# kkaitlyn111/cs336-a2-systems

Measured on AMD Instinct MI355X. Metric: tokens/sec/node GPT-2-XL bf16 DDP, higher is better.
Workload: dtype bf16; 1 GPU; global_batch=102, per_gpu_batch=102, seq_len=512, parallelism=dp1, ddp=none, optimizer=fused HIP AdamW (fp32 master weights), overlapped with backward, attention=HIP FlashAttention-2 (causal), hip_graph=False, gemm_selection=per-problem fastest of hipblaslt default / autotuned lt_gemm / cs336 MFMA GEMM

## Files before the change

csrc/bindings.cpp:

```cpp
#include <ATen/ATen.h>
#include <ATen/hip/HIPContext.h>
#include <c10/core/DeviceGuard.h>
#include <torch/library.h>

#include <algorithm>
#include <cstdlib>
#include <cstring>
#include <mutex>
#include <string>
#include <unordered_map>
#include <vector>

#include "cs336/kernels.h"
#include "../gemm/gemm8.h"

namespace {

using cs336::DType;

DType to_dtype(const at::Tensor& t) {
  switch (t.scalar_type()) {
    case at::kFloat: return DType::F32;
    case at::kBFloat16: return DType::BF16;
    case at::kHalf: return DType::F16;
// ... 903 lines not shown
    TORCH_CHECK(aligned(p) && aligned(g) && aligned(m) && aligned(v) && aligned(s) && aligned(w),
                "cs336: adamw_step_t pointers must be 16-byte aligned");
    const at::Tensor* ts[6] = {&p, &g, &m, &v, &s, &w};
    for (int k = 0; k < 6; ++k) h[(int64_t)i * 6 + k] = reinterpret_cast<int64_t>(ts[k]->data_ptr());
    h[(int64_t)n * 6 + i] = tiles;
    tiles += ((R + 255) / 256) * ((C + 63) / 64);
    int64_t* d = h + (int64_t)n * 6 + (n + 1) + 3 * i;
    d[0] = R;
    d[1] = C;
    d[2] = w.stride(0);
  }
  h[(int64_t)n * 6 + n] = tiles;
  c10::DeviceGuard guard(params[0].device());
  at::Tensor dev = device_table(hv, params[0].device());
  const int64_t* dptr = dev.data_ptr<int64_t>();
  const double alpha_t = lr * (std::sqrt(1.0 - std::pow(beta2, (double)step)) / (1.0 - std::pow(beta1, (double)step)));
  cs336::adamw_step_t(dptr, dptr + (int64_t)n * 6, dptr + (int64_t)n * 6 + (n + 1), n, tiles, to_dtype(grads[0]),
                      (float)beta1, (float)beta2, (float)(1.0 - beta1), (float)(1.0 - beta2), (float)eps,
                      (float)(lr * weight_decay), (float)alpha_t, alpha_ptr(alpha_dev, params[0]), stream());
}

void multi_tensor_cast_bf16(std::vector<at::Tensor> src, std::vector<at::Tensor> dst) {
  if (src.empty()) return;
  check_same_dtype(src, at::kFloat, "src");
  check_same_dtype(dst, at::kBFloat16, "dst");
  c10::DeviceGuard g(src[0].device());
  HostTable ht = build_table({src, dst});
  cs336::multi_tensor_cast_bf16(ht.tt, stream());
}

at::Tensor multi_tensor_l2norm(std::vector<at::Tensor> tensors) {
  TORCH_CHECK(!tensors.empty(), "cs336: empty tensor list");
  const at::ScalarType st = tensors[0].scalar_type();
  check_same_dtype(tensors, st, "tensors");
  c10::DeviceGuard g(tensors[0].device());
  HostTable ht = build_table({tensors});
  at::Tensor partials = at::empty({std::max<int64_t>(ht.tt.total_chunks, 1)}, tensors[0].options().dtype(at::kFloat));
  at::Tensor out = at::zeros({}, tensors[0].options().dtype(at::kFloat));
  cs336::multi_tensor_sumsq(ht.tt, to_dtype(tensors[0]), partials.data_ptr<float>(), stream());
  cs336::finalize_l2norm(partials.data_ptr<float>(), ht.tt.total_chunks, out.data_ptr<float>(), stream());
  return out;
}

void multi_tensor_scale_(std::vector<at::Tensor> tensors, const at::Tensor& scale) {
  if (tensors.empty()) return;
  const at::ScalarType st = tensors[0].scalar_type();
  check_same_dtype(tensors, st, "tensors");
  TORCH_CHECK(scale.scalar_type() == at::kFloat && scale.numel() == 1 && scale.is_cuda(), "cs336: scale");
  c10::DeviceGuard g(tensors[0].device());
  HostTable ht = build_table({tensors});
  cs336::multi_tensor_scale(ht.tt, to_dtype(tensors[0]), scale.data_ptr<float>(), stream());
}

}

void occupy(int64_t n_workgroups, int64_t lds_bytes, double ms, at::Tensor& counter) {
  check_cuda(counter, "counter");
  TORCH_CHECK(counter.scalar_type() == at::kInt && counter.numel() >= 1, "cs336: occupy counter must be int32");
  TORCH_CHECK(n_workgroups > 0 && n_workgroups <= 65536 && lds_bytes >= 4 && lds_bytes <= 160 * 1024 && ms >= 0 &&
                  ms <= 10000,
              "cs336: occupy arguments out of range");
  cs336::occupy((int)n_workgroups, (int)lds_bytes, ms, counter.data_ptr<int>(), stream());
}

void occupy_bytes(int64_t n_workgroups, int64_t lds_bytes, double ms, const at::Tensor& src, at::Tensor& dst,
                  int64_t total_bytes, at::Tensor& counter) {
  check_cuda(src, "src");
  TORCH_CHECK(counter.scalar_type() == at::kInt && counter.numel() >= 1, "cs336: occupy counter must be int32");
  const int64_t nb = src.numel() * src.element_size();
  TORCH_CHECK(src.is_contiguous() && dst.is_contiguous() && dst.numel() * dst.element_size() >= nb && nb >= 16384,
              "cs336: occupy_bytes needs contiguous src/dst of >= 16 KiB, dst at least src's size");
  TORCH_CHECK(n_workgroups > 0 && n_workgroups <= 4096 && lds_bytes >= 4 && lds_bytes <= 65536 && ms > 0 && ms < 10000 &&
                  total_bytes >= 0,
              "cs336: occupy_bytes arguments out of range");
  c10::DeviceGuard g(src.device());
  cs336::occupy_bytes((int)n_workgroups, (int)lds_bytes, ms, src.data_ptr(), dst.data_ptr(), nb & ~(int64_t)16383,
                      total_bytes, counter.data_ptr<int>(), stream());
}

void cohort(int64_t n_workgroups, int64_t lds_bytes, double deadline_ms, at::Tensor& state) {
  check_cuda(state, "state");
  TORCH_CHECK(state.scalar_type() == at::kInt && state.numel() >= 3 && state.is_contiguous(),
              "cs336: cohort state must be a contiguous int32[3]");
  TORCH_CHECK(n_workgroups > 0 && n_workgroups <= 4096 && lds_bytes >= 4 && lds_bytes <= 160 * 1024 &&
                  deadline_ms > 0 && deadline_ms <= 2000,
              "cs336: cohort arguments out of range");
  cs336::cohort((int)n_workgroups, (int)lds_bytes, deadline_ms, state.data_ptr<int>(), stream());
}

bool gemm8_check(const at::Tensor& t, int64_t rows, int64_t cols, const char* what) {
  TORCH_CHECK(t.is_cuda() && t.scalar_type() == at::kBFloat16 && t.dim() == 2 && t.stride(1) == 1, "cs336: gemm8 ",
              what, " must be a row-major bf16 CUDA matrix");
  TORCH_CHECK(t.size(0) == rows && t.size(1) == cols, "cs336: gemm8 ", what, " shape ", t.sizes(), " expected (", rows,
              ", ", cols, ")");
  TORCH_CHECK(t.stride(0) % 8 == 0 && reinterpret_cast<uintptr_t>(t.data_ptr()) % 16 == 0, "cs336: gemm8 ", what,
              " rows must be 16-B aligned");
  return true;
}

bool gemm8_ok(int64_t M, int64_t N, int64_t K, int64_t epi, int64_t half) {
  if (M <= 0 || N <= 0 || K <= 0 || M >= (1 << 30) || N >= (1 << 30) || K >= (1 << 30)) return false;
  const int fn = cs336::gemm8::pick_fn((int)N, (int)epi, (int)half);
  if (fn == 0 || M % 256) return false;
  if (epi == 0) return N % 8 == 0 && K % 8 == 0;
  return K % 64 == 0 && N % (64 * fn) == 0 && (epi != 3 || half % (64 * fn) == 0);
}

constexpr int64_t kDmaLimit = (int64_t(1) << 31) - (int64_t(1) << 20);
bool gemm8_extents_ok(const at::Tensor& a, const at::Tensor& b) {
  const int64_t K = a.size(1);
  return (255 * a.stride(0) + K) * 2 < kDmaLimit && ((b.size(0) - 1) * b.stride(0) + K) * 2 < kDmaLimit;
}

void gemm8(const at::Tensor& a, const at::Tensor& b, at::Tensor& c, int64_t epi, int64_t fn, const OptT& h,
           const OptT& y, int64_t half) {
  const int64_t M = a.size(0), K = a.size(1), N = b.size(0);
  gemm8_check(a, M, K, "a");
  gemm8_check(b, N, K, "b");
  TORCH_CHECK(epi >= 0 && epi <= 2, "cs336: gemm8 epi");
  TORCH_CHECK(gemm8_ok(M, N, K, epi, half), "cs336: gemm8 does not take M=", M, " N=", N, " K=", K, " epi=", epi);
  TORCH_CHECK(gemm8_extents_ok(a, b), "cs336: gemm8 operand extent exceeds the 2 GiB DMA range");
  cs336::gemm8::Args p{};
  p.a = reinterpret_cast<const uint16_t*>(a.data_ptr());
  p.b = reinterpret_cast<const uint16_t*>(b.data_ptr());
  p.lda = a.stride(0);
  p.ldb = b.stride(0);
  p.M = (int)M;
  p.N = (int)N;
  p.K = (int)K;
  p.half = (int)half;
  if (epi == 0) {
    gemm8_check(c, M, N, "c");
  } else if (epi == 1) {
    TORCH_CHECK(N == 2 * half, "cs336: gemm8 epi 1 needs b = [w1; w3] with 2·half rows");
    gemm8_check(c, M, N, "y");
    TORCH_CHECK(h.has_value() && h->defined(), "cs336: gemm8 epi 1 needs h");
    gemm8_check(*h, M, half, "h");
    p.h = reinterpret_cast<uint16_t*>(h->data_ptr());
    p.ldh = h->stride(0);
  } else {
    TORCH_CHECK(N == half, "cs336: gemm8 epi 2 needs b with half rows");
    gemm8_check(c, M, 2 * half, "c = [da|db]");
    TORCH_CHECK(y.has_value() && y->defined(), "cs336: gemm8 epi 2 needs y");
    gemm8_check(*y, M, 2 * half, "y");
    p.y = reinterpret_cast<const uint16_t*>(y->data_ptr());
    p.ldy = y->stride(0);
  }
  p.c = reinterpret_cast<uint16_t*>(c.data_ptr());
  p.ldc = c.stride(0);
  c10::DeviceGuard g(a.device());
  TORCH_CHECK(cs336::gemm8::launch(p, (int)epi, (int)fn, stream()), "cs336: gemm8 launch (fn ", fn, ")");
}

bool gemm8_stamps(const std::optional<at::Tensor>& buf) {
  if (!buf.has_value()) return cs336::gemm8::set_stamp_buffer(nullptr, 0);
  const at::Tensor& b = *buf;
  TORCH_CHECK(b.is_cuda() && b.scalar_type() == at::kLong && b.is_contiguous() && b.dim() == 2 && b.size(1) == 8,
              "cs336: gemm8 stamp buffer must be a contiguous int64 (blocks, 8) GPU tensor");
  return cs336::gemm8::set_stamp_buffer(reinterpret_cast<uint64_t*>(b.data_ptr<int64_t>()), b.size(0));
}

void gemm8_rope(const at::Tensor& a, const at::Tensor& b, at::Tensor& c, const at::Tensor& cos, const at::Tensor& sin,
                const OptT& pos, int64_t seq, int64_t rope_cols, int64_t dhead) {
  const int64_t M = a.size(0), K = a.size(1), N = b.size(0);
  gemm8_check(a, M, K, "a");
  gemm8_check(b, N, K, "b");
  gemm8_check(c, M, N, "c");
  TORCH_CHECK(gemm8_ok(M, N, K, 3, rope_cols), "cs336: gemm8_rope does not take M=", M, " N=", N, " K=", K,
              " rope_cols=", rope_cols);
  TORCH_CHECK(gemm8_extents_ok(a, b), "cs336: gemm8_rope operand extent exceeds the 2 GiB DMA range");
  TORCH_CHECK(dhead % 8 == 0 && dhead > 0 && dhead <= 96 && rope_cols % dhead == 0 && rope_cols <= N && seq > 0,
              "cs336: gemm8_rope needs d_head % 8 == 0, d_head <= 96 and whole rotated heads");
  TORCH_CHECK(cos.is_cuda() && sin.is_cuda() && cos.scalar_type() == at::kFloat && sin.scalar_type() == at::kFloat &&
                  cos.is_contiguous() && sin.is_contiguous() && cos.dim() == 2 && cos.size(1) == dhead / 2 &&
                  sin.sizes() == cos.sizes(),
              "cs336: gemm8_rope cos/sin must be contiguous fp32 (ctx, d_head/2)");
  const int64_t* pp = nullptr;
  if (pos.has_value() && pos->defined()) {
    TORCH_CHECK(pos->is_cuda() && pos->scalar_type() == at::kLong && pos->is_contiguous() && pos->numel() == M,
                "cs336: gemm8_rope pos must be contiguous int64 with one entry per row");
    pp = pos->data_ptr<int64_t>();
  } else {
    TORCH_CHECK(seq <= cos.size(0), "cs336: gemm8_rope seq ", seq, " exceeds the RoPE cache ", cos.size(0));
  }
  cs336::gemm8::Args p{};
  p.a = reinterpret_cast<const uint16_t*>(a.data_ptr());
  p.b = reinterpret_cast<const uint16_t*>(b.data_ptr());
  p.c = reinterpret_cast<uint16_t*>(c.data_ptr());
  p.lda = a.stride(0);
  p.ldb = b.stride(0);
  p.ldc = c.stride(0);
  p.M = (int)M;
  p.N = (int)N;
  p.K = (int)K;
  p.rcos = cos.data_ptr<float>();
  p.rsin = sin.data_ptr<float>();
  p.rpos = pp;
  p.rseq = (int)seq;
  p.rope_cols = (int)rope_cols;
  p.rdh = (int)dhead;
  c10::DeviceGuard g(a.device());
  TORCH_CHECK(cs336::gemm8::launch(p, 3, 0, stream()), "cs336: gemm8_rope launch");
}

void gemm8w(const at::Tensor& a, const at::Tensor& b, at::Tensor& out, int64_t splits, bool trans_out,
            bool accumulate, int64_t fn) {
  TORCH_CHECK(a.is_cuda() && b.is_cuda() && a.scalar_type() == at::kBFloat16 && b.scalar_type() == at::kBFloat16 &&
                  a.dim() == 2 && b.dim() == 2 && a.stride(1) == 1 && b.stride(1) == 1,
              "cs336: gemm8w needs row-major bf16 CUDA operands");
  const int64_t K = a.size(0), M = a.size(1), N = b.size(1);
  TORCH_CHECK(b.size(0) == K, "cs336: gemm8w contraction mismatch");
  TORCH_CHECK(a.stride(0) % 8 == 0 && b.stride(0) % 8 == 0 && reinterpret_cast<uintptr_t>(a.data_ptr()) % 16 == 0 &&
                  reinterpret_cast<uintptr_t>(b.data_ptr()) % 16 == 0 && M % 8 == 0 && N % 8 == 0,
              "cs336: gemm8w needs 16-B aligned rows");
  TORCH_CHECK(out.is_cuda() && out.scalar_type() == at::kFloat, "cs336: gemm8w out must be fp32 CUDA");
  const int64_t rows = trans_out ? N : M, cols = trans_out ? M : N;
  if (splits > 1) {
    TORCH_CHECK(out.dim() == 3 && out.size(0) == splits && out.size(1) == rows && out.size(2) == cols &&
                    out.is_contiguous() && !accumulate,
                "cs336: gemm8w split-K out must be contiguous (splits, rows, cols) slabs");
  } else {
    TORCH_CHECK(out.dim() == 2 && out.size(0) == rows && out.size(1) == cols && out.stride(1) == 1 &&
                    out.stride(0) % 4 == 0 && reinterpret_cast<uintptr_t>(out.data_ptr()) % 16 == 0,
                "cs336: gemm8w out shape/alignment");
  }
  TORCH_CHECK(K % 64 == 0 && K > 0, "cs336: gemm8w needs K % 64 == 0");
  const int64_t ld = std::max(a.stride(0), b.stride(0)), wide = std::max(M, N);
  auto extent = [&](int64_t rows) { return rows * ld * 2 + wide * 2; };
  const int64_t nkt = K / 64, per_split = (nkt + splits - 1) / splits * 64;
  TORCH_CHECK(splits == 1 || extent(per_split) < kDmaLimit, "cs336: gemm8w split of ", per_split,
              " token rows exceeds the 2 GiB DMA range; use more splits (", splits, " given)");
  const int64_t chunk = std::max<int64_t>(64, std::min(K, (kDmaLimit - wide * 2) / (ld * 2) / 64 * 64));
  TORCH_CHECK(splits > 1 || extent(chunk) < kDmaLimit, "cs336: gemm8w rows too wide for the DMA range");
  c10::DeviceGuard g(a.device());
  for (int64_t k0 = 0; k0 < K; k0 += (splits > 1 ? K : chunk)) {
    const int64_t kc = splits > 1 ? K : std::min(chunk, K - k0);
    cs336::gemm8::WArgs p{};
    p.a = reinterpret_cast<const uint16_t*>(a.data_ptr()) + k0 * a.stride(0);
    p.b = reinterpret_cast<const uint16_t*>(b.data_ptr()) + k0 * b.stride(0);
    p.c = out.data_ptr<float>();
    p.lda = a.stride(0);
    p.ldb = b.stride(0);
    p.ldc = splits > 1 ? cols : out.stride(0);
    p.slab_stride = splits > 1 ? rows * cols : 0;
    p.a_elems = (kc - 1) * a.stride(0) + M;
    p.b_elems = (kc - 1) * b.stride(0) + N;
    p.M = (int)M;
    p.N = (int)N;
    p.K = (int)kc;
    p.splits = (int)splits;
    p.trans_out = trans_out ? 1 : 0;
    p.accumulate = (accumulate || k0 > 0) ? 1 : 0;
    TORCH_CHECK(cs336::gemm8::launch_w(p, (int)fn, stream()), "cs336: gemm8w does not take M=", M, " N=", N,
                " K=", kc, " splits=", splits);
  }
}

void splitk_sum(const at::Tensor& slabs, at::Tensor& out, bool accumulate) {
  TORCH_CHECK(slabs.is_cuda() && slabs.scalar_type() == at::kFloat && slabs.dim() == 3 && slabs.is_contiguous(),
              "cs336: splitk_sum slabs must be contiguous fp32 (splits, M, N)");
  const int64_t M = slabs.size(1), N = slabs.size(2);
  TORCH_CHECK(out.is_cuda() && out.scalar_type() == at::kFloat && out.dim() == 2 && out.size(0) == M &&
                  out.size(1) == N && out.stride(1) == 1 && out.stride(0) % 4 == 0 && N % 4 == 0 &&
                  reinterpret_cast<uintptr_t>(out.data_ptr()) % 16 == 0,
              "cs336: splitk_sum out must be fp32 (M, N) with 16-B aligned rows");
  if (M * N == 0 || slabs.size(0) == 0) return;
  c10::DeviceGuard g(slabs.device());
  cs336::gemm::splitk_reduce(slabs.data_ptr<float>(), out.data_ptr<float>(), M, N, (int)slabs.size(0), out.stride(0),
                             accumulate, stream());
}

void check_cache(const at::Tensor& t, const char* name) {
  check_cuda(t, name);
  TORCH_CHECK(t.dim() == 4, "cs336: ", name, " must be (B, H, max_len, D)");
  TORCH_CHECK(t.stride(3) == 1, "cs336: ", name, " must have a contiguous last dim");
  const int64_t es = t.element_size();
  TORCH_CHECK((reinterpret_cast<uintptr_t>(t.data_ptr()) % 16) == 0, "cs336: ", name, " must be 16-byte aligned");
  TORCH_CHECK((t.stride(2) * es) % 16 == 0 && (t.stride(1) * es) % 16 == 0 && (t.stride(0) * es) % 16 == 0,
              "cs336: ", name, " strides must be multiples of 16 bytes");
  TORCH_CHECK(t.stride(0) >= 0 && t.stride(1) >= 0 && t.stride(2) >= t.size(3), "cs336: ", name,
              " rows must not overlap");
  TORCH_CHECK(t.size(2) < ((int64_t)1 << 31), "cs336: ", name, " max_len must fit 32 bits");
}

std::tuple<at::Tensor, at::Tensor> fa_decode(const at::Tensor& q, const at::Tensor& k_cache, const at::Tensor& v_cache,
                                             const at::Tensor& kv_len, double scale, int64_t max_kv_len,
                                             int64_t splits) {
  check_cuda(q, "q");
  check_cache(k_cache, "k_cache");
  check_cache(v_cache, "v_cache");
  TORCH_CHECK(q.dim() == 3, "cs336: fa_decode q must be (B, H, D)");
  const int64_t B = q.size(0), H = q.size(1), D = q.size(2), max_len = k_cache.size(2);
  TORCH_CHECK(D == 32 || D == 64 || D == 80 || D == 128, "cs336: fa_decode head dim must be 32, 64, 80 or 128 (got ", D,
              ")");
  TORCH_CHECK(q.scalar_type() == k_cache.scalar_type() && q.scalar_type() == v_cache.scalar_type(),
              "cs336: q / k_cache / v_cache dtype mismatch");
  TORCH_CHECK(k_cache.sizes() == v_cache.sizes() && k_cache.size(0) == B && k_cache.size(1) == H &&
                  k_cache.size(3) == D,
              "cs336: caches must be (B, H, max_len, D) matching q");
  TORCH_CHECK(k_cache.device() == q.device() && v_cache.device() == q.device() && kv_len.device() == q.device(),
              "cs336: fa_decode tensors must be on one device");
  TORCH_CHECK(kv_len.scalar_type() == at::kInt && kv_len.dim() == 1 && kv_len.size(0) == B && kv_len.is_contiguous(),
              "cs336: kv_len must be a contiguous int32 (B,) device tensor");
  TORCH_CHECK(max_kv_len >= 0 && max_kv_len <= max_len, "cs336: max_kv_len must be in [0, max_len]");
  TORCH_CHECK(splits >= 0 && splits <= 64, "cs336: splits must be in [0, 64] (0 = choose)");
  TORCH_CHECK(B * H * 64 < ((int64_t)1 << 31), "cs336: fa_decode grid too large");
  const DType t = to_dtype(q);
  c10::DeviceGuard g(q.device());
  const at::Tensor qc = q.contiguous();
  TORCH_CHECK((reinterpret_cast<uintptr_t>(qc.data_ptr()) % 16) == 0, "cs336: q must be 16-byte aligned");
  at::Tensor o = at::empty({B, H, D}, q.options());
  at::Tensor lse = at::empty({B, H}, q.options().dtype(at::kFloat));
  if (B * H == 0) return {o, lse};
  cs336::DecodeParams p;
  p.q = qc.data_ptr();
  p.k = k_cache.data_ptr();
  p.v = v_cache.data_ptr();
  p.o = o.data_ptr();
  p.lse = lse.data_ptr<float>();
  p.kv_len = kv_len.data_ptr<int>();
  p.k_sb = k_cache.stride(0); p.k_sh = k_cache.stride(1); p.k_sn = k_cache.stride(2);
  p.v_sb = v_cache.stride(0); p.v_sh = v_cache.stride(1); p.v_sn = v_cache.stride(2);
  p.B = (int)B; p.H = (int)H; p.D = (int)D; p.max_len = (int)max_len;
  p.scale = (float)scale;
  p.splits = splits > 0 ? (int)splits : cs336::fa_decode_splits((int)B, (int)H, (int)D, t, (int)max_kv_len);
  at::Tensor ws;
  if (p.splits > 1) {
    ws = at::empty({(int64_t)p.splits * B * H * (D + 1)}, q.options().dtype(at::kFloat));
    p.opart = ws.data_ptr<float>();
    p.lpart = p.opart + (int64_t)p.splits * B * H * D;
  }
  cs336::fa_decode(p, t, stream());
  return {o, lse};
}

int64_t fa_decode_splits(int64_t B, int64_t H, int64_t D, int64_t elem_size, int64_t max_kv_len) {
  return cs336::fa_decode_splits((int)B, (int)H, (int)D, elem_size == 4 ? DType::F32 : DType::BF16, (int)max_kv_len);
}

at::Tensor kv_append_rope(const at::Tensor& qkv, const at::Tensor& cos, const at::Tensor& sin, const at::Tensor& pos,
                          at::Tensor& k_cache, at::Tensor& v_cache) {
  check_cuda(qkv, "qkv");
  check_cache(k_cache, "k_cache");
  check_cache(v_cache, "v_cache");
  TORCH_CHECK(qkv.dim() == 2 && qkv.stride(1) == 1, "cs336: qkv must be (B, 3*H*D) with a contiguous last dim");
  const int64_t B = k_cache.size(0), H = k_cache.size(1), max_len = k_cache.size(2), D = k_cache.size(3);
  TORCH_CHECK(k_cache.sizes() == v_cache.sizes(), "cs336: k_cache / v_cache shape mismatch");
  TORCH_CHECK(qkv.size(0) == B && qkv.size(1) == 3 * H * D, "cs336: qkv must be (B, 3*H*D) for (B, H, max_len, D) caches");
  TORCH_CHECK(D >= 8 && D <= 256 && D % 8 == 0, "cs336: kv_append_rope head dim must be a multiple of 8 in [8, 256]");
  TORCH_CHECK(qkv.scalar_type() == k_cache.scalar_type() && qkv.scalar_type() == v_cache.scalar_type(),
              "cs336: qkv / k_cache / v_cache dtype mismatch");
  TORCH_CHECK((reinterpret_cast<uintptr_t>(qkv.data_ptr()) % 16) == 0 && (qkv.stride(0) * qkv.element_size()) % 16 == 0 &&
                  qkv.stride(0) >= 0,
              "cs336: qkv rows must be 16-byte aligned");
  TORCH_CHECK(cos.is_cuda() && sin.is_cuda() && cos.scalar_type() == at::kFloat && sin.scalar_type() == at::kFloat &&
                  cos.dim() == 2 && cos.is_contiguous() && sin.is_contiguous() && cos.sizes() == sin.sizes() &&
                  cos.size(1) * 2 == D,
              "cs336: rope cache must be contiguous fp32 (ctx, D/2)");
  TORCH_CHECK(pos.scalar_type() == at::kInt && pos.dim() == 1 && pos.size(0) == B && pos.is_contiguous(),
              "cs336: pos must be a contiguous int32 (B,) device tensor");
  TORCH_CHECK(pos.device() == qkv.device() && cos.device() == qkv.device() && sin.device() == qkv.device() &&
                  k_cache.device() == qkv.device() && v_cache.device() == qkv.device(),
              "cs336: kv_append_rope tensors must be on one device");
  TORCH_CHECK(B * 3 * H * (D / 8) < ((int64_t)1 << 31) && cos.size(0) < ((int64_t)1 << 31),
              "cs336: kv_append_rope too large for 32-bit indexing");
  c10::DeviceGuard g(qkv.device());
  at::Tensor q_out = at::empty({B, H, D}, qkv.options());
  if (B * H == 0) return q_out;
  cs336::AppendParams p;
  p.qkv = qkv.data_ptr();
  p.qkv_sb = qkv.stride(0);
  p.cos = cos.data_ptr<float>();
  p.sin = sin.data_ptr<float>();
  p.pos = pos.data_ptr<int>();
  p.q_out = q_out.data_ptr();
  p.k = k_cache.data_ptr();
  p.v = v_cache.data_ptr();
  p.k_sb = k_cache.stride(0); p.k_sh = k_cache.stride(1); p.k_sn = k_cache.stride(2);
  p.v_sb = v_cache.stride(0); p.v_sh = v_cache.stride(1); p.v_sn = v_cache.stride(2);
  p.B = (int)B; p.H = (int)H; p.D = (int)D; p.max_len = (int)max_len; p.ctx = (int)cos.size(0);
  cs336::kv_append_rope(p, to_dtype(qkv), stream());
  return q_out;
}

bool gemm_skinny_ok(int64_t M, int64_t N, int64_t K, int64_t elem_size) {
  return cs336::gemm_skinny_ok(M, N, K, elem_size);
}

void gemm_skinny(const at::Tensor& x, const at::Tensor& w, at::Tensor& out) {
  check_cuda(x, "x");
  check_cuda(w, "w");
  check_cuda(out, "out");
  TORCH_CHECK(x.dim() == 2 && w.dim() == 2 && out.dim() == 2, "cs336: gemm_skinny takes x (M, K), w (N, K), out (M, N)");
  TORCH_CHECK(x.scalar_type() == at::kBFloat16 || x.scalar_type() == at::kHalf, "cs336: gemm_skinny takes bf16 / fp16");
  TORCH_CHECK(w.scalar_type() == x.scalar_type() && out.scalar_type() == x.scalar_type(),
              "cs336: gemm_skinny x / w / out dtype mismatch");
  TORCH_CHECK(w.device() == x.device() && out.device() == x.device(), "cs336: gemm_skinny tensors must be on one device");
  const int64_t M = x.size(0), K = x.size(1), N = w.size(0);
  TORCH_CHECK(w.size(1) == K && out.size(0) == M && out.size(1) == N, "cs336: gemm_skinny shape mismatch");
  TORCH_CHECK(M >= 1 && M <= 16, "cs336: gemm_skinny takes 1 <= M <= 16 (got ", M, ")");
  TORCH_CHECK(K >= 8 && K % 8 == 0, "cs336: gemm_skinny needs K % 8 == 0 (got ", K, ")");
  TORCH_CHECK(cs336::gemm_skinny_ok(M, N, K, x.element_size()), "cs336: gemm_skinny extents exceed the kernel's 32-bit row / k indices");
  TORCH_CHECK(x.stride(1) == 1 && w.stride(1) == 1 && out.stride(1) == 1, "cs336: gemm_skinny operands must have a contiguous last dim");
  TORCH_CHECK(x.stride(0) % 8 == 0 && (M == 1 || x.stride(0) >= 0), "cs336: gemm_skinny x row stride must be a non-negative multiple of 8");
  TORCH_CHECK(w.stride(0) % 8 == 0 && (N == 1 || w.stride(0) >= K), "cs336: gemm_skinny w row stride must be a multiple of 8, at least K");
// ... 133 lines not shown
```

csrc/gemm/gemm8.h:

```cpp
#pragma once

#include <hip/hip_runtime.h>
#include <stdint.h>

namespace cs336 {
namespace gemm8 {

struct Args {
  const uint16_t* a;
  const uint16_t* b;
  uint16_t* c;
  uint16_t* h;
  const uint16_t* y;
  int64_t lda, ldb, ldc, ldh, ldy;
  int M, N, K;
  int half;
  const float* rcos;
  const float* rsin;
  const int64_t* rpos;
  int rseq, rope_cols, rdh;
  uint64_t* stamps = nullptr;
};
int pick_fn(int N, int epi, int half);
bool set_stamp_buffer(uint64_t* buf, int64_t blocks);
bool launch(const Args& p, int epi, int fn, hipStream_t s);

struct WArgs {
  const uint16_t* a;
  const uint16_t* b;
  float* c;
  int64_t lda, ldb, ldc, slab_stride;
  int64_t a_elems, b_elems;
  int M, N, K;
  int splits;
  int trans_out, accumulate;
};
bool launch_w(const WArgs& p, int fn, hipStream_t s);

}
}
```

csrc/gemm/gemm8w.hip:

```cpp
#include "cs336/kernels.h"
#include "gemm8.h"

namespace cs336 {
namespace gemm8 {
namespace {

typedef __attribute__((ext_vector_type(8))) __bf16 bf16x8;
typedef __attribute__((ext_vector_type(4))) float f32x4;
typedef __attribute__((ext_vector_type(4))) short s16x4;
typedef __attribute__((ext_vector_type(8))) short s16x8;
typedef __attribute__((address_space(3))) s16x4 lds_s16x4;
typedef __attribute__((address_space(3))) void* lds_ptr_t;

constexpr int BM = 256, BK = 64, NT = 512;
constexpr int kGroupM = 8;

__device__ __forceinline__ int xcd_remap(int bid, int total) {
  const int xcd = bid & 7, q = total >> 3, r = total & 7;
  const int base = xcd < r ? xcd * (q + 1) : r * (q + 1) + (xcd - r) * q;
  return base + (bid >> 3);
}
__device__ __forceinline__ void sbarrier() {
  __builtin_amdgcn_sched_barrier(0);
  asm volatile("s_barrier" ::: "memory");
  __builtin_amdgcn_sched_barrier(0);
}
__device__ __forceinline__ void lgkm0() { asm volatile("s_waitcnt lgkmcnt(0)" ::: "memory"); }
template <int N>
__device__ __forceinline__ void vmcnt() {
  asm volatile("s_waitcnt vmcnt(%0)" ::"n"(N) : "memory");
}

template <int S>
__device__ __forceinline__ int swz(int t) {
  static_assert(S % 256 == 0 || S % 256 == 128, "row bytes");
  if constexpr (S % 256 == 0) return (t & 3) | (((t >> 3) & 1) << 2);
  else return ((t >> 1) & 1) | (((t >> 3) & 1) << 1);
}

template <int FN>
struct WGeo {
  static constexpr int BN = 64 * FN, WTN = 16 * FN;
  static constexpr int SA = 2 * BM, SB = 2 * BN;
  static constexpr int A_BYTES = BK * SA, B_BYTES = BK * SB, STAGE = A_BYTES + B_BYTES;
  static constexpr int GA = (32 * SA / 1024) / 8;
  static constexpr int GB_T = 32 * SB / 1024;
  static constexpr int GB_HI = (GB_T + 7) / 8, GB_LO = GB_T / 8;
};

template <int FN, int TRANS>
__global__ __launch_bounds__(NT, 2) void gemm8w_kernel(const WArgs p) {
  using G = WGeo<FN>;
  constexpr int BN = G::BN, WTN = G::WTN, SA = G::SA, SB = G::SB, STAGE = G::STAGE;
  __shared__ __attribute__((aligned(1024))) char smem[2 * STAGE];

  const int tid = threadIdx.x, lane = tid & 63;
  const int wave = __builtin_amdgcn_readfirstlane(tid >> 6);
  const int wr = wave >> 2, wc = wave & 3;

  const int tiles_n = p.N / BN, tiles_m = (p.M + BM - 1) / BM;
  const int bid = xcd_remap(blockIdx.x, gridDim.x);
  const int per_group = kGroupM * tiles_n;
  const int first_m = (bid / per_group) * kGroupM;
  const int gsz = min(tiles_m - first_m, kGroupM);
  const int tm = first_m + (bid % per_group) % gsz, tn = (bid % per_group) / gsz;
  const int m0 = tm * BM, n0 = tn * BN;

  const int nkt_all = p.K / BK, split = blockIdx.y, nsplit = gridDim.y;
  const int kt0 = (int)((int64_t)nkt_all * split / nsplit), kt1 = (int)((int64_t)nkt_all * (split + 1) / nsplit);
  const int nkt = kt1 - kt0;

  const int64_t a_off = (int64_t)kt0 * BK * p.lda + m0, b_off = (int64_t)kt0 * BK * p.ldb + n0;
  auto rec = [](int64_t elems) -> uint32_t {
    const int64_t bytes = elems > 0 ? 2 * elems : 0;
    return (uint32_t)(bytes < 0x7fffffff ? bytes : 0x7fffffff);
  };
  const uint32_t a_rec = rec(p.a_elems - a_off), b_rec = rec(p.b_elems - b_off);
  const __amdgpu_buffer_rsrc_t ra = __builtin_amdgcn_make_buffer_rsrc((void*)(p.a + a_off), (short)0, a_rec, 0x00020000);
  const __amdgpu_buffer_rsrc_t rb = __builtin_amdgcn_make_buffer_rsrc((void*)(p.b + b_off), (short)0, b_rec, 0x00020000);

  uint32_t va[2][G::GA], la[2][G::GA];
  uint32_t vb[2][G::GB_HI], lb[2][G::GB_HI];
  auto src_off = [&](int S, int64_t ld, int byte) -> uint32_t {
    const int t = byte / S, cb = byte % S, ps = cb >> 5, hb = (cb >> 4) & 1;
    const int ls = ps ^ (S == SA ? swz<SA>(t) : swz<SB>(t));
    return 2u * (uint32_t)(t * ld + ls * 16 + hb * 8);
  };
#pragma unroll
  for (int h = 0; h < 2; ++h) {
#pragma unroll
    for (int i = 0; i < G::GA; ++i) {
      const int g = wave + 8 * i;
      const int byte = h * 32 * SA + g * 1024;
      la[h][i] = (uint32_t)byte;
      va[h][i] = src_off(SA, p.lda, byte + lane * 16);
    }
#pragma unroll
    for (int i = 0; i < G::GB_HI; ++i) {
      int g;
      if constexpr (G::GB_HI == G::GB_LO) g = wave + 8 * i;
      else g = (wr == h) ? (wc + 4 * i) : (12 + wc + 4 * i);
      const int byte = h * 32 * SB + g * 1024;
      lb[h][i] = (uint32_t)(G::A_BYTES + byte);
      vb[h][i] = src_off(SB, p.ldb, byte + lane * 16);
    }
  }
  const int nb_h0 = (G::GB_HI == G::GB_LO || wr == 0) ? G::GB_HI : G::GB_LO;
  const int nb_h1 = (G::GB_HI == G::GB_LO || wr == 1) ? G::GB_HI : G::GB_LO;
  const uint32_t lds_base = (uint32_t)(uintptr_t)(lds_ptr_t)smem;
  auto glds = [&](const __amdgpu_buffer_rsrc_t& rs, uint32_t vo, uint32_t so, uint32_t lds_off) {
    asm volatile("s_mov_b32 m0, %1\n\ts_nop 0\n\tbuffer_load_dwordx4 %0, %2, %3 offen lds"
                 :
                 : "v"(vo), "s"(lds_base + lds_off), "s"(rs), "s"(so)
                 : "memory");
  };
#define CS336_G8W_ISSUE(H, KT, ST)                                                                          \
  do {                                                                                                     \
    const uint32_t base_ = (uint32_t)((ST) * STAGE);                                                       \
    const uint32_t soa_ = (uint32_t)(KT) * BK * 2u * (uint32_t)p.lda, sob_ = (uint32_t)(KT) * BK * 2u * (uint32_t)p.ldb; \
    _Pragma("unroll") for (int i_ = 0; i_ < G::GA; ++i_)                                                   \
      glds(ra, va[H][i_], soa_, base_ + la[H][i_]); \
    const int nb_ = (H) == 0 ? nb_h0 : nb_h1;                                                              \
    _Pragma("unroll") for (int i_ = 0; i_ < G::GB_HI; ++i_) if (i_ < nb_)                                  \
      glds(rb, vb[H][i_], sob_, base_ + lb[H][i_]); \
  } while (0)
  const bool big0 = G::GB_HI != G::GB_LO && wr == 0;
  constexpr int N01 = 2 * G::GA + G::GB_HI + G::GB_LO;

  const int g4 = lane >> 4, q = (lane >> 2) & 3, pp = lane & 3;
  auto tr = [&](uint32_t img, int S, int c0, int t) -> s16x4 {
    const int s = c0 >> 4, f = S == SA ? swz<SA>(t) : swz<SB>(t);
    const uint32_t off = img + (uint32_t)(t * S + ((s ^ f) << 5) + 8 * pp);
    return __builtin_amdgcn_ds_read_tr16_b64_v4i16((lds_s16x4*)(smem + off));
  };
  auto frag = [&](uint32_t img, int S, int c0, int ks) -> bf16x8 {
    const int t0 = 32 * ks + 8 * g4 + q;
    const s16x4 lo = tr(img, S, c0, t0), hi = tr(img, S, c0, t0 + 4);
    return __builtin_bit_cast(bf16x8, __builtin_shufflevector(lo, hi, 0, 1, 2, 3, 4, 5, 6, 7));
  };

  f32x4 acc[8][FN];
#pragma unroll
  for (int i = 0; i < 8; ++i)
#pragma unroll
    for (int j = 0; j < FN; ++j) acc[i][j] = f32x4{0.f, 0.f, 0.f, 0.f};
  bf16x8 fa[4], fb[FN];
  const int arow = wr * 128, bcol = wc * WTN;
  auto wait_a = [&]() { lgkm0(); };
  auto wait_ab = [&]() { lgkm0(); };

  auto mma = [&](int i0) {
    __builtin_amdgcn_s_setprio(1);
#pragma unroll
    for (int i = 0; i < 4; ++i)
#pragma unroll
      for (int j = 0; j < FN; ++j) {
        if constexpr (TRANS)
          acc[i0 + i][j] = __builtin_amdgcn_mfma_f32_16x16x32_bf16(fa[i], fb[j], acc[i0 + i][j], 0, 0, 0);
        else
          acc[i0 + i][j] = __builtin_amdgcn_mfma_f32_16x16x32_bf16(fb[j], fa[i], acc[i0 + i][j], 0, 0, 0);
      }
    __builtin_amdgcn_s_setprio(0);
  };

  if (nkt > 0) {
    CS336_G8W_ISSUE(0, 0, 0);
    CS336_G8W_ISSUE(1, 0, 0);
    if (nkt > 1) {
      CS336_G8W_ISSUE(0, 1, 1);
      vmcnt<N01>();
    } else {
      if (big0) vmcnt<G::GA + G::GB_LO>();
      else vmcnt<G::GA + G::GB_HI>();
    }
  }
  sbarrier();
  if (wr == 1) sbarrier();

  for (int t = 0; t < nkt; ++t) {
    const uint32_t st = (uint32_t)((t & 1) * STAGE);
    if (t + 1 < nkt) CS336_G8W_ISSUE(1, t + 1, (t + 1) & 1);
#pragma unroll
    for (int i = 0; i < 4; ++i) fa[i] = frag(st, SA, arow + 16 * i, 0);
#pragma unroll
    for (int j = 0; j < FN; ++j) fb[j] = frag(st + G::A_BYTES, SB, bcol + 16 * j, 0);
    wait_ab();
    sbarrier();
    mma(0);
    sbarrier();
#pragma unroll
    for (int i = 0; i < 4; ++i) fa[i] = frag(st, SA, arow + 64 + 16 * i, 0);
    if (t + 1 < nkt) vmcnt<N01>();
    else vmcnt<0>();
    wait_a();
    sbarrier();
    mma(4);
    sbarrier();
    if (t + 2 < nkt) CS336_G8W_ISSUE(0, t + 2, t & 1);
#pragma unroll
    for (int i = 0; i < 4; ++i) fa[i] = frag(st, SA, arow + 16 * i, 1);
#pragma unroll
    for (int j = 0; j < FN; ++j) fb[j] = frag(st + G::A_BYTES, SB, bcol + 16 * j, 1);
    wait_ab();
    sbarrier();
    mma(0);
    sbarrier();
#pragma unroll
    for (int i = 0; i < 4; ++i) fa[i] = frag(st, SA, arow + 64 + 16 * i, 1);
    if (t + 1 < nkt) {
      if (t + 2 < nkt) {
        vmcnt<N01>();
      } else if (big0) {
        vmcnt<G::GA + G::GB_LO>();
      } else {
        vmcnt<G::GA + G::GB_HI>();
      }
    }
    wait_a();
    sbarrier();
    mma(4);
    sbarrier();
  }
#undef CS336_G8W_ISSUE
  if (wr == 0) sbarrier();

  float* c = p.c + (int64_t)split * p.slab_stride;
  const int lr = lane & 15, lq = 4 * (lane >> 4);
#pragma unroll
  for (int i = 0; i < 8; ++i)
#pragma unroll
    for (int j = 0; j < FN; ++j) {
      const f32x4 v = acc[i][j];
      if constexpr (TRANS) {
        const int m = m0 + arow + 16 * i + lq, n = n0 + bcol + 16 * j + lr;
        if (m < p.M) {
          float4* d = reinterpret_cast<float4*>(c + (int64_t)n * p.ldc + m);
          float4 w = make_float4(v[0], v[1], v[2], v[3]);
          if (p.accumulate) {
            const float4 o = *d;
            w.x += o.x; w.y += o.y; w.z += o.z; w.w += o.w;
          }
          *d = w;
        }
      } else {
        const int m = m0 + arow + 16 * i + lr, n = n0 + bcol + 16 * j + lq;
        if (m < p.M) {
          float4* d = reinterpret_cast<float4*>(c + (int64_t)m * p.ldc + n);
          float4 w = make_float4(v[0], v[1], v[2], v[3]);
          if (p.accumulate) {
            const float4 o = *d;
            w.x += o.x; w.y += o.y; w.z += o.z; w.w += o.w;
          }
          *d = w;
        }
      }
    }
}

template <int FN, int TRANS>
void launch_wt(const WArgs& p, hipStream_t s) {
  const dim3 grid((unsigned)(((p.M + BM - 1) / BM) * (p.N / (64 * FN))), (unsigned)p.splits), block(NT);
  hipLaunchKernelGGL((gemm8w_kernel<FN, TRANS>), grid, block, 0, s, p);
}

}

bool launch_w(const WArgs& p, int fn, hipStream_t s) {
  if (p.K % BK || p.K < BK || p.M <= 0 || p.M % 4 || p.splits < 1 || p.splits > 64) return false;
  if (fn == 0) fn = p.N % 320 == 0 ? 5 : (p.N % 256 == 0 ? 4 : 0);
  if ((fn != 4 && fn != 5) || p.N % (64 * fn)) return false;
  if (p.splits > 1 && p.accumulate) return false;
  if (fn == 5) {
    if (p.trans_out) launch_wt<5, 1>(p, s);
    else launch_wt<5, 0>(p, s);
  } else {
    if (p.trans_out) launch_wt<4, 1>(p, s);
    else launch_wt<4, 0>(p, s);
  }
  return true;
}

}
}
```

Baseline: 88730 tokens/s.

## Restructure gemm8w K-loop into two full-tile phases with precomputed LDS addresses

The weight-gradient GEMM main loop now reads all eight A fragments and all B fragments per k-substep, then issues one 8xFN MFMA block, replacing four half-tile phases with two. LDS read addresses are precomputed once per thread and advanced by a stage offset each tile, so the swizzle arithmetic leaves the inner loop. This halves the barrier count per tile but holds more fragments in registers, which may raise VGPR pressure. Optional compile-time timestamp instrumentation is also added, with the stamp buffer threaded through WArgs.

```diff
diff --git a/csrc/bindings.cpp b/csrc/bindings.cpp
--- a/csrc/bindings.cpp
+++ b/csrc/bindings.cpp
@@ -1079,12 +1079,18 @@
   TORCH_CHECK(cs336::gemm8::launch(p, (int)epi, (int)fn, stream()), "cs336: gemm8 launch (fn ", fn, ")");
 }
 
+uint64_t* g_stamp_buf = nullptr;
+int64_t g_stamp_rows = 0;
 bool gemm8_stamps(const std::optional<at::Tensor>& buf) {
+  g_stamp_buf = nullptr;
+  g_stamp_rows = 0;
   if (!buf.has_value()) return cs336::gemm8::set_stamp_buffer(nullptr, 0);
   const at::Tensor& b = *buf;
   TORCH_CHECK(b.is_cuda() && b.scalar_type() == at::kLong && b.is_contiguous() && b.dim() == 2 && b.size(1) == 8,
               "cs336: gemm8 stamp buffer must be a contiguous int64 (blocks, 8) GPU tensor");
-  return cs336::gemm8::set_stamp_buffer(reinterpret_cast<uint64_t*>(b.data_ptr<int64_t>()), b.size(0));
+  g_stamp_buf = reinterpret_cast<uint64_t*>(b.data_ptr<int64_t>());
+  g_stamp_rows = b.size(0);
+  return cs336::gemm8::set_stamp_buffer(g_stamp_buf, g_stamp_rows);
 }
 
 void gemm8_rope(const at::Tensor& a, const at::Tensor& b, at::Tensor& c, const at::Tensor& cos, const at::Tensor& sin,
@@ -1178,6 +1184,8 @@
     p.splits = (int)splits;
     p.trans_out = trans_out ? 1 : 0;
     p.accumulate = (accumulate || k0 > 0) ? 1 : 0;
+    p.stamps = g_stamp_buf;
+    p.stamp_rows = g_stamp_rows;
     TORCH_CHECK(cs336::gemm8::launch_w(p, (int)fn, stream()), "cs336: gemm8w does not take M=", M, " N=", N,
                 " K=", kc, " splits=", splits);
   }
diff --git a/csrc/gemm/gemm8.h b/csrc/gemm/gemm8.h
--- a/csrc/gemm/gemm8.h
+++ b/csrc/gemm/gemm8.h
@@ -34,6 +34,8 @@
   int M, N, K;
   int splits;
   int trans_out, accumulate;
+  uint64_t* stamps = nullptr;
+  int64_t stamp_rows = 0;
 };
 bool launch_w(const WArgs& p, int fn, hipStream_t s);
 
diff --git a/csrc/gemm/gemm8w.hip b/csrc/gemm/gemm8w.hip
--- a/csrc/gemm/gemm8w.hip
+++ b/csrc/gemm/gemm8w.hip
@@ -128,14 +128,19 @@
   constexpr int N01 = 2 * G::GA + G::GB_HI + G::GB_LO;
 
   const int g4 = lane >> 4, q = (lane >> 2) & 3, pp = lane & 3;
-  auto tr = [&](uint32_t img, int S, int c0, int t) -> s16x4 {
-    const int s = c0 >> 4, f = S == SA ? swz<SA>(t) : swz<SB>(t);
-    const uint32_t off = img + (uint32_t)(t * S + ((s ^ f) << 5) + 8 * pp);
-    return __builtin_amdgcn_ds_read_tr16_b64_v4i16((lds_s16x4*)(smem + off));
-  };
-  auto frag = [&](uint32_t img, int S, int c0, int ks) -> bf16x8 {
-    const int t0 = 32 * ks + 8 * g4 + q;
-    const s16x4 lo = tr(img, S, c0, t0), hi = tr(img, S, c0, t0 + 4);
+  uint32_t ada[8], adb[FN];
+  {
+    const int t0 = 8 * g4 + q;
+#pragma unroll
+    for (int i = 0; i < 8; ++i)
+      ada[i] = (uint32_t)(t0 * SA + ((((wr * 128 + 16 * i) >> 4) ^ swz<SA>(t0)) << 5) + 8 * pp);
+#pragma unroll
+    for (int j = 0; j < FN; ++j)
+      adb[j] = (uint32_t)(G::A_BYTES + t0 * SB + ((((wc * WTN + 16 * j) >> 4) ^ swz<SB>(t0)) << 5) + 8 * pp);
+  }
+  auto frag = [&](uint32_t addr, int S, int ks) -> bf16x8 {
+    const s16x4 lo = __builtin_amdgcn_ds_read_tr16_b64_v4i16((lds_s16x4*)(smem + addr + 32 * ks * S));
+    const s16x4 hi = __builtin_amdgcn_ds_read_tr16_b64_v4i16((lds_s16x4*)(smem + addr + 32 * ks * S + 4 * S));
     return __builtin_bit_cast(bf16x8, __builtin_shufflevector(lo, hi, 0, 1, 2, 3, 4, 5, 6, 7));
   };
 
@@ -144,23 +149,79 @@
   for (int i = 0; i < 8; ++i)
 #pragma unroll
     for (int j = 0; j < FN; ++j) acc[i][j] = f32x4{0.f, 0.f, 0.f, 0.f};
-  bf16x8 fa[4], fb[FN];
+  bf16x8 fx[4], fy[4], fb[FN];
   const int arow = wr * 128, bcol = wc * WTN;
-  auto wait_a = [&]() { lgkm0(); };
-  auto wait_ab = [&]() { lgkm0(); };
-
-  auto mma = [&](int i0) {
+
+  auto mma = [&]() {
     __builtin_amdgcn_s_setprio(1);
 #pragma unroll
-    for (int i = 0; i < 4; ++i)
+    for (int i = 0; i < 8; ++i)
 #pragma unroll
       for (int j = 0; j < FN; ++j) {
+        const bf16x8& a = i < 4 ? fx[i & 3] : fy[i & 3];
         if constexpr (TRANS)
-          acc[i0 + i][j] = __builtin_amdgcn_mfma_f32_16x16x32_bf16(fa[i], fb[j], acc[i0 + i][j], 0, 0, 0);
+          acc[i][j] = __builtin_amdgcn_mfma_f32_16x16x32_bf16(a, fb[j], acc[i][j], 0, 0, 0);
         else
-          acc[i0 + i][j] = __builtin_amdgcn_mfma_f32_16x16x32_bf16(fb[j], fa[i], acc[i0 + i][j], 0, 0, 0);
+          acc[i][j] = __builtin_amdgcn_mfma_f32_16x16x32_bf16(fb[j], a, acc[i][j], 0, 0, 0);
       }
     __builtin_amdgcn_s_setprio(0);
+  };
+  auto read_x = [&](int ks) {
+#pragma unroll
+    for (int i = 0; i < 4; ++i) fx[i] = frag(ada[i], SA, ks);
+  };
+  auto read_y = [&](int ks) {
+#pragma unroll
+    for (int i = 0; i < 4; ++i) fy[i] = frag(ada[4 + i], SA, ks);
+  };
+  auto read_b = [&](int ks) {
+#pragma unroll
+    for (int j = 0; j < FN; ++j) fb[j] = frag(adb[j], SB, ks);
+  };
+  auto next_stage = [&](int t) {
+    const uint32_t d = (t & 1) ? (uint32_t)(-STAGE) : (uint32_t)STAGE;
+#pragma unroll
+    for (int i = 0; i < 8; ++i) {
+      ada[i] += d;
+      asm volatile("" : "+v"(ada[i]));
+    }
+#pragma unroll
+    for (int j = 0; j < FN; ++j) {
+      adb[j] += d;
+      asm volatile("" : "+v"(adb[j]));
+    }
+  };
+
+#ifdef CS336_G8_STAMP
+  constexpr int kStampTiles = 4, kPhases = 2;
+  const int s_lo = nkt > kStampTiles ? (nkt - kStampTiles) / 2 : 0;
+  uint32_t s_work[4] = {0, 0, 0, 0}, s_wait[4] = {0, 0, 0, 0}, s_mma[4] = {0, 0, 0, 0}, s_cnt = 0;
+  auto stamp = [&]() -> uint32_t {
+    uint64_t v;
+    __builtin_amdgcn_sched_barrier(0);
+    asm volatile("s_memtime %0\n\ts_waitcnt lgkmcnt(0)" : "=s"(v)::"memory");
+    __builtin_amdgcn_sched_barrier(0);
+    return (uint32_t)v;
+  };
+#define CS336_G8W_STAMP(I) \
+  do {                     \
+    if (samp) ts_[I] = stamp(); \
+  } while (0)
+#else
+#define CS336_G8W_STAMP(I) \
+  do {                     \
+  } while (0)
+#endif
+
+  auto wait_h1 = [&](bool more1) {
+    if (more1) vmcnt<N01>();
+    else vmcnt<0>();
+  };
+  auto wait_h0 = [&](bool more1, bool more2) {
+    if (!more1) return;
+    if (more2) vmcnt<N01>();
+    else if (big0) vmcnt<G::GA + G::GB_LO>();
+    else vmcnt<G::GA + G::GB_HI>();
   };
 
   if (nkt > 0) {
@@ -178,51 +239,67 @@
   if (wr == 1) sbarrier();
 
   for (int t = 0; t < nkt; ++t) {
-    const uint32_t st = (uint32_t)((t & 1) * STAGE);
-    if (t + 1 < nkt) CS336_G8W_ISSUE(1, t + 1, (t + 1) & 1);
-#pragma unroll
-    for (int i = 0; i < 4; ++i) fa[i] = frag(st, SA, arow + 16 * i, 0);
-#pragma unroll
-    for (int j = 0; j < FN; ++j) fb[j] = frag(st + G::A_BYTES, SB, bcol + 16 * j, 0);
-    wait_ab();
+    const bool more1 = t + 1 < nkt, more2 = t + 2 < nkt;
+#ifdef CS336_G8_STAMP
+    const bool samp = t >= s_lo && t < s_lo + kStampTiles;
+    uint32_t ts_[3 * kPhases + 1] = {};
+#endif
+    CS336_G8W_STAMP(0);
+    if (more1) CS336_G8W_ISSUE(1, t + 1, (t + 1) & 1);
+    read_x(0);
+    read_y(0);
+    read_b(0);
+    wait_h1(more1);
+    lgkm0();
+    CS336_G8W_STAMP(1);
     sbarrier();
-    mma(0);
+    CS336_G8W_STAMP(2);
+    mma();
     sbarrier();
-#pragma unroll
-    for (int i = 0; i < 4; ++i) fa[i] = frag(st, SA, arow + 64 + 16 * i, 0);
-    if (t + 1 < nkt) vmcnt<N01>();
-    else vmcnt<0>();
-    wait_a();
+    CS336_G8W_STAMP(3);
+    if (more2) CS336_G8W_ISSUE(0, t + 2, t & 1);
+    read_x(1);
+    read_y(1);
+    read_b(1);
+    wait_h0(more1, more2);
+    lgkm0();
+    CS336_G8W_STAMP(4);
     sbarrier();
-    mma(4);
+    CS336_G8W_STAMP(5);
+    mma();
+    next_stage(t);
     sbarrier();
-    if (t + 2 < nkt) CS336_G8W_ISSUE(0, t + 2, t & 1);
-#pragma unroll
-    for (int i = 0; i < 4; ++i) fa[i] = frag(st, SA, arow + 16 * i, 1);
-#pragma unroll
-    for (int j = 0; j < FN; ++j) fb[j] = frag(st + G::A_BYTES, SB, bcol + 16 * j, 1);
-    wait_ab();
-    sbarrier();
-    mma(0);
-    sbarrier();
-#pragma unroll
-    for (int i = 0; i < 4; ++i) fa[i] = frag(st, SA, arow + 64 + 16 * i, 1);
-    if (t + 1 < nkt) {
-      if (t + 2 < nkt) {
-        vmcnt<N01>();
-      } else if (big0) {
-        vmcnt<G::GA + G::GB_LO>();
-      } else {
-        vmcnt<G::GA + G::GB_HI>();
+    CS336_G8W_STAMP(6);
+#ifdef CS336_G8_STAMP
+    if (samp) {
+#pragma unroll
+      for (int ph = 0; ph < kPhases; ++ph) {
+        s_work[ph] += ts_[3 * ph + 1] - ts_[3 * ph];
+        s_wait[ph] += ts_[3 * ph + 2] - ts_[3 * ph + 1];
+        s_mma[ph] += ts_[3 * ph + 3] - ts_[3 * ph + 2];
       }
-    }
-    wait_a();
-    sbarrier();
-    mma(4);
-    sbarrier();
+      ++s_cnt;
+    }
+#endif
   }
 #undef CS336_G8W_ISSUE
+#undef CS336_G8W_STAMP
   if (wr == 0) sbarrier();
+#ifdef CS336_G8_STAMP
+  if (p.stamps && lane == 0 && wc == 0) {
+    uint32_t hw, xcc;
+    asm volatile("s_getreg_b32 %0, hwreg(HW_REG_HW_ID)" : "=s"(hw));
+    asm volatile("s_getreg_b32 %0, hwreg(HW_REG_XCC_ID)" : "=s"(xcc));
+    uint64_t* o = p.stamps + 32 * ((int64_t)blockIdx.y * gridDim.x + blockIdx.x) + 16 * wr;
+#pragma unroll
+    for (int ph = 0; ph < kPhases; ++ph) {
+      o[ph] = s_work[ph];
+      o[4 + ph] = s_wait[ph];
+      o[8 + ph] = s_mma[ph];
+    }
+    o[12] = s_cnt; o[13] = (uint64_t)nkt; o[14] = hw; o[15] = xcc;
+  }
+#endif
 
   float* c = p.c + (int64_t)split * p.slab_stride;
   const int lr = lane & 15, lq = 4 * (lane >> 4);
@@ -258,8 +335,10 @@
 }
 
 template <int FN, int TRANS>
-void launch_wt(const WArgs& p, hipStream_t s) {
+void launch_wt(const WArgs& p_in, hipStream_t s) {
+  WArgs p = p_in;
   const dim3 grid((unsigned)(((p.M + BM - 1) / BM) * (p.N / (64 * FN))), (unsigned)p.splits), block(NT);
+  if (4 * (int64_t)grid.x * grid.y > p.stamp_rows) p.stamps = nullptr;
   hipLaunchKernelGGL((gemm8w_kernel<FN, TRANS>), grid, block, 0, s, p);
 }
 
```

After: 90510 tokens/s, median of 6. 2.0% higher.
